# yetanotherco/yet-another-halo2-fork

Hardware: AMD Instinct MI355X
Metric: create_proof wall-seconds at k=22 (BN254/KZG); MSM Mscalar-mul/s at 2^24 (lower is better)
Workload: dtype u32 limbs (BN254 Fr/Fq Montgomery, 256-bit modular integer)

## Files before the change

yet-another-halo2-fork_amd/csrc/f29.h:

```cpp
#pragma once
#include "bn254.h"

namespace h2g {

static constexpr uint32_t F29_MASK = (1u << 29) - 1;

H2G_HD constexpr uint32_t limb29_of(const uint32_t* x, int i, int sh) {
  const int b = 29 * i - sh;
  if (b < 0) return (x[0] << (-b)) & F29_MASK;
  const int w = b >> 5, s = b & 31;
  const uint64_t lo = w < 8 ? x[w] : 0;
  const uint64_t hi = w + 1 < 8 ? x[w + 1] : 0;
  return (uint32_t)(((hi << 32) | lo) >> s) & F29_MASK;
}
template <class P>
struct C29 {
  static constexpr uint32_t M[9] = {limb29_of(P::M, 0, 0), limb29_of(P::M, 1, 0), limb29_of(P::M, 2, 0),
                                    limb29_of(P::M, 3, 0), limb29_of(P::M, 4, 0), limb29_of(P::M, 5, 0),
                                    limb29_of(P::M, 6, 0), limb29_of(P::M, 7, 0), limb29_of(P::M, 8, 0)};
  static constexpr uint32_t INV = P::INV & F29_MASK;
  static constexpr uint32_t ONE256[9] = {limb29_of(P::ONE, 0, 0), limb29_of(P::ONE, 1, 0), limb29_of(P::ONE, 2, 0),
                                         limb29_of(P::ONE, 3, 0), limb29_of(P::ONE, 4, 0), limb29_of(P::ONE, 5, 0),
                                         limb29_of(P::ONE, 6, 0), limb29_of(P::ONE, 7, 0), limb29_of(P::ONE, 8, 0)};
};

struct F29 {
  uint32_t l[9];
};

struct Limbs9 {
  uint32_t v[9];
};
template <class P>
constexpr Limbs9 kmul_norm(uint32_t k) {
  Limbs9 r{};
  uint64_t c = 0;
  for (int i = 0; i < 9; i++) {
    const uint64_t t = (uint64_t)limb29_of(P::M, i, 0) * k + c;
    r.v[i] = i < 8 ? (uint32_t)(t & F29_MASK) : (uint32_t)t;
    c = t >> 29;
  }
  return r;
}
template <class P>
constexpr uint32_t kmul_safe(uint32_t k, int off, int i) {
  const Limbs9 n = kmul_norm<P>(k);
  const uint32_t unit = 1u << (off - 29);
  if (i == 0) return n.v[0] + (1u << off);
  if (i < 8) return n.v[i] + (1u << off) - unit;
  return n.v[8] - unit;
}
template <class P, uint32_t K, int OFF>
struct KM29 {
  static constexpr uint32_t L[9] = {kmul_safe<P>(K, OFF, 0), kmul_safe<P>(K, OFF, 1), kmul_safe<P>(K, OFF, 2),
                                    kmul_safe<P>(K, OFF, 3), kmul_safe<P>(K, OFF, 4), kmul_safe<P>(K, OFF, 5),
                                    kmul_safe<P>(K, OFF, 6), kmul_safe<P>(K, OFF, 7), kmul_safe<P>(K, OFF, 8)};
};
template <class P>
constexpr Limbs9 one29() {
  Limbs9 r{};
  for (int i = 0; i < 9; i++) r.v[i] = limb29_of(P::ONE, i, 5);
  for (int it = 0; it < 40; it++) {
    bool ge = true;
    for (int i = 8; i >= 0; i--) {
      const uint32_t m = limb29_of(P::M, i, 0);
      if (r.v[i] != m) {
        ge = r.v[i] > m;
        break;
      }
    }
    if (!ge) break;
    int64_t br = 0;
    for (int i = 0; i < 9; i++) {
      int64_t t = (int64_t)r.v[i] - limb29_of(P::M, i, 0) + br;
      br = t < 0 ? -1 : 0;
      r.v[i] = (uint32_t)(t & F29_MASK);
    }
  }
  return r;
}
template <class P>
struct One29 {
  static constexpr Limbs9 v = one29<P>();
  static constexpr uint32_t L[9] = {v.v[0], v.v[1], v.v[2], v.v[3], v.v[4], v.v[5], v.v[6], v.v[7], v.v[8]};
};

template <class P>
H2G_HD F29 to29(const Fe<P>& x) {
  F29 r;
  r.l[0] = (x.l[0] << 5) & F29_MASK;
#pragma unroll
  for (int i = 1; i < 9; i++) {
    const int b = 29 * i - 5, w = b >> 5, s = b & 31;
    const uint64_t lo = x.l[w];
    const uint64_t hi = w + 1 < 8 ? x.l[w + 1] : 0;
    r.l[i] = (uint32_t)(((hi << 32) | lo) >> s) & F29_MASK;
  }
  return r;
}

template <class P>
H2G_HD F29 mul29(const F29& a, const F29& b) {
  uint32_t m[9];
  F29 r;
  uint64_t acc = 0;
#pragma unroll
  for (int k = 0; k < 9; k++) {
    uint64_t acc2 = 0;
#pragma unroll
    for (int i = 0; i <= k; i++) acc += (uint64_t)a.l[i] * b.l[k - i];
#pragma unroll
    for (int i = 0; i < k; i++) acc2 += (uint64_t)m[i] * C29<P>::M[k - i];
    acc += acc2;
    m[k] = ((uint32_t)acc * C29<P>::INV) & F29_MASK;
    acc += (uint64_t)m[k] * C29<P>::M[0];
    acc >>= 29;
  }
#pragma unroll
  for (int k = 9; k < 17; k++) {
    uint64_t acc2 = 0;
#pragma unroll
    for (int i = k - 8; i < 9; i++) {
      acc += (uint64_t)a.l[i] * b.l[k - i];
      acc2 += (uint64_t)m[i] * C29<P>::M[k - i];
    }
    acc += acc2;
    r.l[k - 9] = (uint32_t)acc & F29_MASK;
    acc >>= 29;
  }
  r.l[8] = (uint32_t)acc;
  return r;
}

template <class P>
H2G_HD F29 sqr29(const F29& a) {
  uint32_t m[9], d[9];
#pragma unroll
  for (int i = 0; i < 9; i++) d[i] = a.l[i] << 1;
  F29 r;
  uint64_t acc = 0;
#pragma unroll
  for (int k = 0; k < 17; k++) {
#pragma unroll
    for (int i = (k > 8 ? k - 8 : 0); 2 * i < k; i++) acc += (uint64_t)d[i] * a.l[k - i];
    if ((k & 1) == 0) acc += (uint64_t)a.l[k / 2] * a.l[k / 2];
    if (k < 9) {
#pragma unroll
      for (int i = 0; i < k; i++) acc += (uint64_t)m[i] * C29<P>::M[k - i];
      m[k] = ((uint32_t)acc * C29<P>::INV) & F29_MASK;
      acc += (uint64_t)m[k] * C29<P>::M[0];
    } else {
#pragma unroll
      for (int i = k - 8; i < 9; i++) acc += (uint64_t)m[i] * C29<P>::M[k - i];
      r.l[k - 9] = (uint32_t)acc & F29_MASK;
    }
    acc >>= 29;
  }
  r.l[8] = (uint32_t)acc;
  return r;
}

template <class P>
H2G_HD Fe<P> from29(const F29& v) {
  F29 k;
#pragma unroll
  for (int i = 0; i < 9; i++) k.l[i] = C29<P>::ONE256[i];
  const F29 t = mul29<P>(v, k);
  Fe<P> r;
  uint64_t acc = 0;
  int have = 0, w = 0;
#pragma unroll
  for (int i = 0; i < 9; i++) {
    acc |= (uint64_t)t.l[i] << have;
    have += 29;
    if (have >= 32 && w < 8) {
      r.l[w++] = (uint32_t)acc;
      acc >>= 32;
      have -= 32;
    }
  }
  if (w < 8) r.l[w] = (uint32_t)acc;
  return reduce_once(r);
}


H2G_HD F29 add29(const F29& a, const F29& b) {
  F29 r;
#pragma unroll
  for (int i = 0; i < 9; i++) r.l[i] = a.l[i] + b.l[i];
  return r;
}
template <class P, uint32_t K, int OFF>
H2G_HD F29 sub29(const F29& a, const F29& b) {
  F29 r;
#pragma unroll
  for (int i = 0; i < 9; i++) r.l[i] = (a.l[i] + KM29<P, K, OFF>::L[i]) - b.l[i];
  return r;
}
H2G_HD F29 norm29(F29 a) {
#pragma unroll
  for (int i = 0; i < 8; i++) {
    a.l[i + 1] += a.l[i] >> 29;
    a.l[i] &= F29_MASK;
  }
  return a;
}

template <class P>
H2G_HD F29 mul29x2(const F29& a, const F29& b, const F29& c, const F29& d) {
  uint32_t m[9];
  F29 r;
  uint64_t acc = 0;
#pragma unroll
  for (int k = 0; k < 9; k++) {
#pragma unroll
    for (int i = 0; i <= k; i++) {
      acc += (uint64_t)a.l[i] * b.l[k - i];
      acc += (uint64_t)c.l[i] * d.l[k - i];
    }
#pragma unroll
    for (int i = 0; i < k; i++) acc += (uint64_t)m[i] * C29<P>::M[k - i];
    m[k] = ((uint32_t)acc * C29<P>::INV) & F29_MASK;
    acc += (uint64_t)m[k] * C29<P>::M[0];
    acc >>= 29;
  }
#pragma unroll
  for (int k = 9; k < 17; k++) {
#pragma unroll
    for (int i = k - 8; i < 9; i++) {
      acc += (uint64_t)a.l[i] * b.l[k - i];
      acc += (uint64_t)c.l[i] * d.l[k - i];
      acc += (uint64_t)m[i] * C29<P>::M[k - i];
    }
    r.l[k - 9] = (uint32_t)acc & F29_MASK;
    acc >>= 29;
  }
  r.l[8] = (uint32_t)acc;
  return r;
}

template <class P>
H2G_HD bool is_zero29(const F29& a) {
  constexpr uint32_t minv = (0u - C29<P>::INV) & F29_MASK;
  const uint32_t k = (a.l[0] * minv) & F29_MASK;
  if (k > 1024) return false;
  uint64_t c = 0;
  uint32_t diff = 0;
#pragma unroll
  for (int i = 0; i < 9; i++) {
    const uint64_t t = (uint64_t)C29<P>::M[i] * k + c;
    const uint32_t limb = i < 8 ? (uint32_t)(t & F29_MASK) : (uint32_t)t;
    c = t >> 29;
    diff |= limb ^ a.l[i];
  }
  return diff == 0;
}
template <class P>
H2G_HD F29 one29v() {
  F29 r;
#pragma unroll
  for (int i = 0; i < 9; i++) r.l[i] = One29<P>::L[i];
  return r;
}

struct G1xyzz29 {
  F29 X, Y, ZZ, ZZZ;
};
H2G_HD G1xyzz29 xyzz29_identity() {
  G1xyzz29 r;
#pragma unroll
  for (int i = 0; i < 9; i++) r.X.l[i] = r.Y.l[i] = r.ZZ.l[i] = r.ZZZ.l[i] = 0;
  return r;
}
H2G_HD bool xyzz29_is_identity(const G1xyzz29& p) {
  uint32_t z = 0;
#pragma unroll
  for (int i = 0; i < 9; i++) z |= p.ZZ.l[i];
  return z == 0;
}
template <class P = FqParams>
H2G_HD G1xyzz xyzz_from29(const G1xyzz29& p) {
  G1xyzz r;
  r.X = from29<FqParams>(p.X);
  r.Y = from29<FqParams>(p.Y);
  r.ZZ = from29<FqParams>(p.ZZ);
  r.ZZZ = from29<FqParams>(p.ZZZ);
  return r;
}
template <class P>
H2G_HD F29 to29_reduced(const Fe<P>& v) {
  return mul29<P>(to29(v), one29v<P>());
}
H2G_HD G1xyzz29 xyzz29_from_xyzz(const G1xyzz& p) {
  G1xyzz29 r;
  r.X = to29_reduced(p.X);
  r.Y = to29_reduced(p.Y);
  r.ZZ = to29_reduced(p.ZZ);
  r.ZZZ = to29_reduced(p.ZZZ);
  return r;
}

template <bool DBL = true>
H2G_HD G1xyzz29 xyzz29_madd(const G1xyzz29& p, const F29& qx, const F29& qy, bool* dbl = nullptr) {
  using P = FqParams;
  if (xyzz29_is_identity(p)) {
    G1xyzz29 r;
    r.X = qx;
    r.Y = qy;
    r.ZZ = one29v<P>();
    r.ZZZ = r.ZZ;
    return r;
  }
  const F29 U2 = mul29<P>(qx, p.ZZ);
  const F29 S2 = mul29<P>(qy, p.ZZZ);
  const F29 Pp = norm29(sub29<P, 64, 29>(U2, p.X));
  const F29 R = norm29(sub29<P, 64, 29>(S2, p.Y));
  if (is_zero29<P>(Pp)) {
    if (is_zero29<P>(R)) {
      if constexpr (DBL) {
        G1Affine a;
        a.x = from29<P>(qx);
        a.y = from29<P>(qy);
        return xyzz29_from_xyzz(xyzz_mdbl(a));
      } else {
        *dbl = true;
      }
    }
    return xyzz29_identity();
  }
  const F29 PP = sqr29<P>(Pp);
  const F29 PPP = mul29<P>(Pp, PP);
  const F29 Q = mul29<P>(p.X, PP);
  const F29 R2 = sqr29<P>(R);
  G1xyzz29 r;
  r.X = norm29(sub29<P, 32, 31>(R2, add29(add29(PPP, Q), Q)));
  r.Y = mul29x2<P>(R, sub29<P, 64, 29>(Q, r.X), p.Y, sub29<P, 16, 29>(F29{}, PPP));
  r.ZZ = mul29<P>(p.ZZ, PP);
  r.ZZZ = mul29<P>(p.ZZZ, PPP);
  return r;
}


template <class P>
H2G_HD F29 raw29(const Fe<P>& x) {
  F29 r;
#pragma unroll
  for (int i = 0; i < 9; i++) {
    const int b = 29 * i, w = b >> 5, s = b & 31;
    const uint64_t lo = x.l[w];
    const uint64_t hi = w + 1 < 8 ? x.l[w + 1] : 0;
    r.l[i] = (uint32_t)(((hi << 32) | lo) >> s) & F29_MASK;
  }
  return r;
}
template <class P>
H2G_HD Fe<P> pack29(const F29& v) {
  Fe<P> r;
  uint64_t acc = 0;
  int have = 0, w = 0;
#pragma unroll
  for (int i = 0; i < 9; i++) {
    acc |= (uint64_t)v.l[i] << have;
    have += 29;
    if (have >= 32 && w < 8) {
      r.l[w++] = (uint32_t)acc;
      acc >>= 32;
      have -= 32;
    }
  }
  if (w < 8) r.l[w] = (uint32_t)acc;
  return r;
}
template <class P>
H2G_HD F29 sub_m_if_ge29(const F29& v) {
  F29 d;
  int32_t br = 0;
#pragma unroll
  for (int i = 0; i < 9; i++) {
    const int32_t t = (int32_t)v.l[i] - (int32_t)C29<P>::M[i] + br;
    if (i < 8) {
      d.l[i] = (uint32_t)t & F29_MASK;
      br = t >> 29;
    } else {
      d.l[i] = (uint32_t)t;
      br = t >> 31;
    }
  }
  F29 r;
#pragma unroll
  for (int i = 0; i < 9; i++) r.l[i] = br ? v.l[i] : d.l[i];
  return r;
}
template <class P>
H2G_HD Fe<P> storage_to_f29_packed(const Fe<P>& s) {
  return pack29<P>(sub_m_if_ge29<P>(mul29<P>(to29(s), one29v<P>())));
}
template <class P>
H2G_HD F29 storage_to_f29(const Fe<P>& s) {
  return sub_m_if_ge29<P>(mul29<P>(to29(s), one29v<P>()));
}



template <class P>
H2G_HD F29 reduce29(const F29& v) {
  constexpr uint32_t mt = C29<P>::M[8] + 1;
  const uint32_t q = v.l[8] / mt;
  F29 r;
  int64_t br = 0;
#pragma unroll
  for (int i = 0; i < 9; i++) {
    const int64_t t = (int64_t)v.l[i] - (int64_t)((uint64_t)q * C29<P>::M[i]) + br;
    if (i < 8) {
      r.l[i] = (uint32_t)t & F29_MASK;
      br = t >> 29;
    } else {
      r.l[i] = (uint32_t)t;
    }
  }
  return r;
}
H2G_HD G1xyzz29 xyzz29_reduce(const G1xyzz29& p) {
  G1xyzz29 r;
  r.X = reduce29<FqParams>(p.X);
  r.Y = reduce29<FqParams>(p.Y);
  r.ZZ = reduce29<FqParams>(p.ZZ);
  r.ZZZ = reduce29<FqParams>(p.ZZZ);
  return r;
}

H2G_HD G1xyzz29 xyzz29_dbl(const G1xyzz29& p) {
  using P = FqParams;
  if (xyzz29_is_identity(p)) return p;
  const F29 U = norm29(add29(p.Y, p.Y));
  const F29 V = sqr29<P>(U);
  const F29 W = mul29<P>(U, V);
  const F29 S = mul29<P>(p.X, V);
  const F29 X2 = sqr29<P>(p.X);
  const F29 Mm = norm29(add29(add29(X2, X2), X2));
  G1xyzz29 r;
  r.X = reduce29<P>(norm29(sub29<P, 4, 31>(sqr29<P>(Mm), add29(S, S))));
  r.Y = mul29x2<P>(Mm, sub29<P, 4, 29>(S, r.X), p.Y, sub29<P, 2, 29>(F29{}, W));
  r.ZZ = mul29<P>(V, p.ZZ);
  r.ZZZ = mul29<P>(W, p.ZZZ);
  return r;
}

H2G_HD G1xyzz29 xyzz29_add(const G1xyzz29& p, const G1xyzz29& q) {
  using P = FqParams;
  if (xyzz29_is_identity(q)) return p;
  if (xyzz29_is_identity(p)) return q;
  const F29 U1 = mul29<P>(p.X, q.ZZ);
  const F29 U2 = mul29<P>(q.X, p.ZZ);
  const F29 S1 = mul29<P>(p.Y, q.ZZZ);
  const F29 S2 = mul29<P>(q.Y, p.ZZZ);
  const F29 Pp = norm29(sub29<P, 2, 29>(U2, U1));
  const F29 R = norm29(sub29<P, 2, 29>(S2, S1));
  if (is_zero29<P>(Pp)) {
    if (is_zero29<P>(R)) return xyzz29_dbl(p);
    return xyzz29_identity();
  }
  const F29 PP = sqr29<P>(Pp);
  const F29 PPP = mul29<P>(Pp, PP);
  const F29 Q = mul29<P>(U1, PP);
  G1xyzz29 r;
  r.X = reduce29<P>(norm29(sub29<P, 4, 31>(sqr29<P>(R), add29(add29(PPP, Q), Q))));
  r.Y = mul29x2<P>(R, sub29<P, 4, 29>(Q, r.X), S1, sub29<P, 2, 29>(F29{}, PPP));
  r.ZZ = mul29<P>(mul29<P>(p.ZZ, q.ZZ), PP);
  r.ZZZ = mul29<P>(mul29<P>(p.ZZZ, q.ZZZ), PPP);
  return r;
}

H2G_HD G1xyzz29 xyzz29_mul_u32(const G1xyzz29& p, uint32_t k) {
  if (k == 0) return xyzz29_identity();
  int top = 31;
  while (!((k >> top) & 1)) top--;
  G1xyzz29 acc = p;
  for (int b = top - 1; b >= 0; b--) {
    acc = xyzz29_dbl(acc);
    if ((k >> b) & 1) acc = xyzz29_add(acc, p);
  }
  return acc;
}

}
```

yet-another-halo2-fork_amd/csrc/msm_acc.hip:

```cpp
#include "msm_part.h"

namespace h2g {

static constexpr int MSM_THREADS = 256;

__device__ __forceinline__ G1Affine ld_aff(const G1Affine* p) {
  const uint4* q = reinterpret_cast<const uint4*>(p);
  uint4 a = q[0], b = q[1], c = q[2], d = q[3];
  G1Affine r;
  r.x.l[0] = a.x; r.x.l[1] = a.y; r.x.l[2] = a.z; r.x.l[3] = a.w;
  r.x.l[4] = b.x; r.x.l[5] = b.y; r.x.l[6] = b.z; r.x.l[7] = b.w;
  r.y.l[0] = c.x; r.y.l[1] = c.y; r.y.l[2] = c.z; r.y.l[3] = c.w;
  r.y.l[4] = d.x; r.y.l[5] = d.y; r.y.l[6] = d.z; r.y.l[7] = d.w;
  return r;
}

__device__ __forceinline__ void msm_emit(uint32_t key, const AccPoint& acc, bool first, bool from_prev, bool to_next,
                                         uint32_t t, AccPoint* __restrict__ buckets, AccPoint* __restrict__ bnd) {
  AccPoint* dst = (!from_prev && !to_next) ? buckets + key : bnd + 2 * (size_t)t + (first ? 0 : 1);
  st_acc(dst, acc);
}

__device__ __forceinline__ AccPoint acc_identity() { return xyzz29_identity(); }
template <bool SAFE>
__device__ __forceinline__ AccPoint acc_madd(const AccPoint& acc, const G1Affine& pt, bool* dbl) {
  if (pt.is_identity()) return acc;
  return xyzz29_madd<SAFE>(acc, to29(pt.x), to29(pt.y), dbl);
}

template <bool SAFE>
__device__ __forceinline__ bool acc_chunk(uint32_t t, const G1Affine* __restrict__ bases,
                                          const uint32_t* __restrict__ vals, const uint32_t* __restrict__ koff,
                                          uint32_t nbt, uint32_t total, uint32_t L, AccPoint* __restrict__ buckets,
                                          AccPoint* __restrict__ bnd) {
  const uint32_t lo = t * L;
  if (lo >= total) return false;
  const uint32_t hi = lo + L < total ? lo + L : total;
  uint32_t key = 0, kh = nbt;
  while (kh - key > 1) {
    const uint32_t mid = (key + kh) >> 1;
    if (koff[mid] <= lo) key = mid;
    else kh = mid;
  }
  const bool prev_same = koff[key] < lo;
  uint32_t kend = koff[key + 1];
  bool first = true, dbl = false;
  AccPoint acc = acc_identity();
  uint32_t v = vals[lo];
  G1Affine pt = ld_aff(bases + (v & 0x7fffffffu));
  for (uint32_t p = lo; p < hi; p++) {
    const uint32_t v_next = vals[p + 1 < hi ? p + 1 : p];
    const G1Affine pt_next = ld_aff(bases + (v_next & 0x7fffffffu));
    if (p == kend) {
      msm_emit(key, acc, first, first && prev_same, false, t, buckets, bnd);
      first = false;
      uint32_t a = key + 1, b = a + 1, step = 1;
      while (b < nbt && koff[b] <= p) {
        a = b;
        step <<= 1;
        b = a + step;
      }
      if (b > nbt) b = nbt;
      while (b - a > 1) {
        const uint32_t mid = (a + b) >> 1;
        if (koff[mid] <= p) a = mid;
        else b = mid;
      }
      key = a;
      kend = koff[key + 1];
      acc = acc_identity();
    }
    if (v >> 31) pt = affine_neg(pt);
    acc = acc_madd<SAFE>(acc, pt, &dbl);
    v = v_next;
    pt = pt_next;
  }
  msm_emit(key, acc, first, first && prev_same, kend > hi, t, buckets, bnd);
  return dbl;
}

__global__ void __launch_bounds__(MSM_THREADS)
msm_acc_kernel(const G1Affine* __restrict__ bases, const uint32_t* __restrict__ vals,
               const uint32_t* __restrict__ koff, uint32_t nbt, const uint32_t* __restrict__ d_total,
               AccPoint* __restrict__ buckets, AccPoint* __restrict__ bnd, uint32_t* __restrict__ rep) {
  const uint32_t t = blockIdx.x * blockDim.x + threadIdx.x;
  if (acc_chunk<false>(t, bases, vals, koff, nbt, d_total[0], d_total[1], buckets, bnd)) {
    const uint32_t i = atomicAdd(rep, 1u);
    if (i < MSM_REPAIR_CAP) rep[1 + i] = t;
  }
}

__global__ void __launch_bounds__(MSM_THREADS)
msm_acc_repair_kernel(const G1Affine* __restrict__ bases, const uint32_t* __restrict__ vals,
                      const uint32_t* __restrict__ koff, uint32_t nbt, const uint32_t* __restrict__ d_total,
                      AccPoint* __restrict__ buckets, AccPoint* __restrict__ bnd, const uint32_t* __restrict__ rep) {
  const uint32_t cnt = rep[0];
  if (cnt == 0) return;
  const uint32_t total = d_total[0], L = d_total[1], nchunks = (total + L - 1) / L;
  const uint32_t g = blockIdx.x * blockDim.x + threadIdx.x, stride = gridDim.x * blockDim.x;
  if (cnt <= MSM_REPAIR_CAP) {
    for (uint32_t i = g; i < cnt; i += stride) (void)acc_chunk<true>(rep[1 + i], bases, vals, koff, nbt, total, L,
                                                                      buckets, bnd);
  } else {
    for (uint32_t t = g; t < nchunks; t += stride) (void)acc_chunk<true>(t, bases, vals, koff, nbt, total, L, buckets,
                                                                         bnd);
  }
}

hipError_t msm_accumulate(const G1Affine* bases, const uint32_t* vals, const uint32_t* koff, uint32_t nbt,
                          const uint32_t* d_total, size_t nchunks_cap, AccPoint* buckets, AccPoint* bnd,
                          uint32_t* rep, hipStream_t st) {
  const int T = MSM_THREADS;
  const unsigned cgrid = (unsigned)((nchunks_cap + T - 1) / T);
  hipLaunchKernelGGL(msm_acc_kernel, dim3(cgrid), dim3(T), 0, st, bases, vals, koff, nbt, d_total, buckets, bnd, rep);
  hipLaunchKernelGGL(msm_acc_repair_kernel, dim3(MSM_REPAIR_BLOCKS), dim3(T), 0, st, bases, vals, koff, nbt, d_total,
                     buckets, bnd, (const uint32_t*)rep);
  return hipGetLastError();
}

}
```

Measured before the change: 0.07460.

## Use fused-accumulator Montgomery mul/sqr and in-place XYZZ madd in MSM accumulation

Adds 29-bit-limb Montgomery multiply, square and dual-multiply routines that run product and reduction through one 64-bit accumulator. An empty asm constraint pins that accumulator to vector registers. An in-place XYZZ mixed-add uses them, reports equal or doubling cases as a status code, and uses normalized-constant subtraction. The fast accumulation path now loads the first point of each bucket run directly instead of adding it to the identity, tracks identity with a flag, and sets launch bounds to four waves per SIMD. This targets field-arithmetic instruction count and register pressure in the hot madd loop. The register cap risks spills, and the SAFE path now calls xyzz29_madd without the doubling pointer, which only compiles if a matching overload exists.

Result: faster. 0.07335 (median of 6 runs) (-1.7%).

```diff
diff --git a/yet-another-halo2-fork_amd/csrc/f29.h b/yet-another-halo2-fork_amd/csrc/f29.h
--- a/yet-another-halo2-fork_amd/csrc/f29.h
+++ b/yet-another-halo2-fork_amd/csrc/f29.h
@@ -341,6 +341,142 @@
 }
 
 
+#if defined(__HIP_DEVICE_COMPILE__)
+#define H2G_PIN64(x) asm("" : "+v"(x))
+#else
+#define H2G_PIN64(x) ((void)0)
+#endif
+#define H2G_MAC(acc, x, y)          \
+  do {                              \
+    acc += (uint64_t)(x) * (y);     \
+    H2G_PIN64(acc);                 \
+  } while (0)
+template <class P>
+H2G_HD F29 mul29_acc(const F29& a, const F29& b) {
+  uint32_t m[9];
+  F29 r;
+  uint64_t acc = 0;
+#pragma unroll
+  for (int k = 0; k < 17; k++) {
+    const int i0 = k > 8 ? k - 8 : 0, i1 = k > 8 ? 8 : k;
+    H2G_MAC(acc, a.l[i0], b.l[k - i0]);
+#pragma unroll
+    for (int i = i0 + 1; i <= i1; i++) H2G_MAC(acc, a.l[i], b.l[k - i]);
+    if (k < 9) {
+#pragma unroll
+      for (int i = 0; i < k; i++) H2G_MAC(acc, m[i], C29<P>::M[k - i]);
+      m[k] = ((uint32_t)acc * C29<P>::INV) & F29_MASK;
+      H2G_MAC(acc, m[k], C29<P>::M[0]);
+    } else {
+#pragma unroll
+      for (int i = k - 8; i < 9; i++) H2G_MAC(acc, m[i], C29<P>::M[k - i]);
+      r.l[k - 9] = (uint32_t)acc & F29_MASK;
+    }
+    acc >>= 29;
+  }
+  r.l[8] = (uint32_t)acc;
+  return r;
+}
+template <class P>
+H2G_HD F29 sqr29_acc(const F29& a) {
+  uint32_t m[9], d[9];
+#pragma unroll
+  for (int i = 0; i < 9; i++) d[i] = a.l[i] << 1;
+  F29 r;
+  uint64_t acc = 0;
+#pragma unroll
+  for (int k = 0; k < 17; k++) {
+    const int i0 = k > 8 ? k - 8 : 0;
+    if (2 * i0 < k) H2G_MAC(acc, d[i0], a.l[k - i0]);
+    else H2G_MAC(acc, a.l[k / 2], a.l[k / 2]);
+#pragma unroll
+    for (int i = i0 + 1; 2 * i < k; i++) H2G_MAC(acc, d[i], a.l[k - i]);
+    if ((k & 1) == 0 && 2 * i0 < k) H2G_MAC(acc, a.l[k / 2], a.l[k / 2]);
+    if (k < 9) {
+#pragma unroll
+      for (int i = 0; i < k; i++) H2G_MAC(acc, m[i], C29<P>::M[k - i]);
+      m[k] = ((uint32_t)acc * C29<P>::INV) & F29_MASK;
+      H2G_MAC(acc, m[k], C29<P>::M[0]);
+    } else {
+#pragma unroll
+      for (int i = k - 8; i < 9; i++) H2G_MAC(acc, m[i], C29<P>::M[k - i]);
+      r.l[k - 9] = (uint32_t)acc & F29_MASK;
+    }
+    acc >>= 29;
+  }
+  r.l[8] = (uint32_t)acc;
+  return r;
+}
+template <class P>
+H2G_HD F29 mul29x2_acc(const F29& a, const F29& b, const F29& c, const F29& d) {
+  uint32_t m[9];
+  F29 r;
+  uint64_t acc = 0;
+#pragma unroll
+  for (int k = 0; k < 17; k++) {
+    const int i0 = k > 8 ? k - 8 : 0, i1 = k > 8 ? 8 : k;
+    H2G_MAC(acc, a.l[i0], b.l[k - i0]);
+    H2G_MAC(acc, c.l[i0], d.l[k - i0]);
+#pragma unroll
+    for (int i = i0 + 1; i <= i1; i++) {
+      H2G_MAC(acc, a.l[i], b.l[k - i]);
+      H2G_MAC(acc, c.l[i], d.l[k - i]);
+    }
+    if (k < 9) {
+#pragma unroll
+      for (int i = 0; i < k; i++) H2G_MAC(acc, m[i], C29<P>::M[k - i]);
+      m[k] = ((uint32_t)acc * C29<P>::INV) & F29_MASK;
+      H2G_MAC(acc, m[k], C29<P>::M[0]);
+    } else {
+#pragma unroll
+      for (int i = k - 8; i < 9; i++) H2G_MAC(acc, m[i], C29<P>::M[k - i]);
+      r.l[k - 9] = (uint32_t)acc & F29_MASK;
+    }
+    acc >>= 29;
+  }
+  r.l[8] = (uint32_t)acc;
+  return r;
+}
+
+template <class P, uint32_t K>
+struct KMN29 {
+  static constexpr Limbs9 n = kmul_norm<P>(K);
+  static constexpr uint32_t L[9] = {n.v[0], n.v[1], n.v[2], n.v[3], n.v[4], n.v[5], n.v[6], n.v[7], n.v[8]};
+};
+template <class P, uint32_t K>
+H2G_HD F29 subn29(const F29& a, const F29& b) {
+  F29 r;
+  int32_t c = 0;
+#pragma unroll
+  for (int i = 0; i < 8; i++) {
+    const int32_t t = (int32_t)(a.l[i] - b.l[i]) + (int32_t)KMN29<P, K>::L[i] + c;
+    r.l[i] = (uint32_t)t & F29_MASK;
+    c = t >> 29;
+  }
+  r.l[8] = (a.l[8] - b.l[8]) + KMN29<P, K>::L[8] + (uint32_t)c;
+  return r;
+}
+
+H2G_HD int xyzz29_madd_acc(G1xyzz29& p, const F29& qx, const F29& qy) {
+  using P = FqParams;
+  const F29 U2 = mul29_acc<P>(qx, p.ZZ);
+  const F29 S2 = mul29_acc<P>(qy, p.ZZZ);
+  const F29 Pp = subn29<P, 64>(U2, p.X);
+  const F29 R = subn29<P, 64>(S2, p.Y);
+  int st = 0;
+  if (is_zero29<P>(Pp)) st = is_zero29<P>(R) ? 2 : 1;
+  const F29 PP = sqr29_acc<P>(Pp);
+  const F29 Q = mul29_acc<P>(p.X, PP);
+  const F29 PPP = mul29_acc<P>(Pp, PP);
+  p.ZZ = mul29_acc<P>(p.ZZ, PP);
+  p.ZZZ = mul29_acc<P>(p.ZZZ, PPP);
+  const F29 R2 = sqr29_acc<P>(R);
+  p.X = subn29<P, 32>(R2, add29(add29(PPP, Q), Q));
+  p.Y = mul29x2_acc<P>(R, sub29<P, 64, 29>(Q, p.X), p.Y, sub29<P, 16, 29>(F29{}, PPP));
+  return st;
+}
+
+
 template <class P>
 H2G_HD F29 raw29(const Fe<P>& x) {
   F29 r;
diff --git a/yet-another-halo2-fork_amd/csrc/msm_acc.hip b/yet-another-halo2-fork_amd/csrc/msm_acc.hip
--- a/yet-another-halo2-fork_amd/csrc/msm_acc.hip
+++ b/yet-another-halo2-fork_amd/csrc/msm_acc.hip
@@ -15,18 +15,15 @@
   return r;
 }
 
-__device__ __forceinline__ void msm_emit(uint32_t key, const AccPoint& acc, bool first, bool from_prev, bool to_next,
-                                         uint32_t t, AccPoint* __restrict__ buckets, AccPoint* __restrict__ bnd) {
+__device__ __forceinline__ void msm_emit(uint32_t key, const AccPoint& acc, bool ident, bool first, bool from_prev,
+                                         bool to_next, uint32_t t, AccPoint* __restrict__ buckets,
+                                         AccPoint* __restrict__ bnd) {
   AccPoint* dst = (!from_prev && !to_next) ? buckets + key : bnd + 2 * (size_t)t + (first ? 0 : 1);
-  st_acc(dst, acc);
+  if (ident) st_acc(dst, xyzz29_identity());
+  else st_acc(dst, acc);
 }
 
 __device__ __forceinline__ AccPoint acc_identity() { return xyzz29_identity(); }
-template <bool SAFE>
-__device__ __forceinline__ AccPoint acc_madd(const AccPoint& acc, const G1Affine& pt, bool* dbl) {
-  if (pt.is_identity()) return acc;
-  return xyzz29_madd<SAFE>(acc, to29(pt.x), to29(pt.y), dbl);
-}
 
 template <bool SAFE>
 __device__ __forceinline__ bool acc_chunk(uint32_t t, const G1Affine* __restrict__ bases,
@@ -44,7 +41,7 @@
   }
   const bool prev_same = koff[key] < lo;
   uint32_t kend = koff[key + 1];
-  bool first = true, dbl = false;
+  bool first = true, dbl = false, fresh = true;
   AccPoint acc = acc_identity();
   uint32_t v = vals[lo];
   G1Affine pt = ld_aff(bases + (v & 0x7fffffffu));
@@ -52,7 +49,7 @@
     const uint32_t v_next = vals[p + 1 < hi ? p + 1 : p];
     const G1Affine pt_next = ld_aff(bases + (v_next & 0x7fffffffu));
     if (p == kend) {
-      msm_emit(key, acc, first, first && prev_same, false, t, buckets, bnd);
+      msm_emit(key, acc, !SAFE && fresh, first, first && prev_same, false, t, buckets, bnd);
       first = false;
       uint32_t a = key + 1, b = a + 1, step = 1;
       while (b < nbt && koff[b] <= p) {
@@ -68,18 +65,36 @@
       }
       key = a;
       kend = koff[key + 1];
-      acc = acc_identity();
+      if constexpr (SAFE) acc = acc_identity();
+      fresh = true;
     }
     if (v >> 31) pt = affine_neg(pt);
-    acc = acc_madd<SAFE>(acc, pt, &dbl);
+    if constexpr (SAFE) {
+      if (!pt.is_identity()) acc = xyzz29_madd<true>(acc, to29(pt.x), to29(pt.y));
+    } else {
+      const bool skip = pt.is_identity(), start = fresh;
+      const F29 qx = to29(pt.x), qy = to29(pt.y);
+      if (!skip && start) {
+        acc.X = qx;
+        acc.Y = qy;
+        acc.ZZ = one29v<FqParams>();
+        acc.ZZZ = acc.ZZ;
+        fresh = false;
+      }
+      if (!skip && !start) {
+        const int st = xyzz29_madd_acc(acc, qx, qy);
+        fresh = st != 0;
+        dbl |= st == 2;
+      }
+    }
     v = v_next;
     pt = pt_next;
   }
-  msm_emit(key, acc, first, first && prev_same, kend > hi, t, buckets, bnd);
+  msm_emit(key, acc, !SAFE && fresh, first, first && prev_same, kend > hi, t, buckets, bnd);
   return dbl;
 }
 
-__global__ void __launch_bounds__(MSM_THREADS)
+__global__ void __launch_bounds__(MSM_THREADS, 4)
 msm_acc_kernel(const G1Affine* __restrict__ bases, const uint32_t* __restrict__ vals,
                const uint32_t* __restrict__ koff, uint32_t nbt, const uint32_t* __restrict__ d_total,
                AccPoint* __restrict__ buckets, AccPoint* __restrict__ bnd, uint32_t* __restrict__ rep) {
```
